# zhuduowang/Change3D

Hardware: AMD Instinct MI355X
Metric: train images/sec (256x256 pairs, X3D-L BCD) (higher is better)
Workload: dtype bf16; 1 GPU; BCD X3D-L bf16, B=32/GPU, 256x256 synthetic LEVIR-CD-shaped pairs, T=3, train step (fwd+BCE/Dice+bwd+Adam); global_batch=32, parallelism=dp1, dist_world_size=1, hip_graph=False, full=False, settle_steps=40, input=resident in HBM

## Files before the change

change3d_amd/_lib.py:

```python
import ctypes as C
import os

_HERE = os.path.dirname(os.path.abspath(__file__))
LIB_PATH = os.environ.get("C3D_LIB") or os.path.join(_HERE, "lib", "libchange3d_hip.so")

DT_F32, DT_BF16 = 0, 1
PRO_NONE, PRO_BN_SE_SWISH, PRO_AFFINE2 = 0, 1, 2
EPI_STORE, EPI_STATS, EPI_SWISH_SE_BWD, EPI_ADD = 0, 1, 2, 3
AUG_NONE, AUG_BCD, AUG_SCD, AUG_BDA = 0, 1, 2, 3
ROWS_DENSE, ROWS_FRAME, ROWS_STRIDE2, ROWS_S2SHIFT = 0, 1, 2, 3
SC_NONE, SC_IDENTITY, SC_BN, SC_RAW = 0, 1, 2, 3
STAT_STRIPES = 16
OPT_SIDE_STREAM, OPT_STEM_MFMA, OPT_CONVT_MFMA, OPT_FUSE_WGRAD, OPT_FOLD_SE, OPT_MASK_IN_DGRAD, OPT_DW_RING, OPT_PW_WGRAD_V2, OPT_DW_FWD_HV, OPT_PW_CFWD, OPT_PW_CDG, OPT_DW_T4 = 0, 1, 2, 3, 4, 5, 6, 7, 8, 9, 10, 11
STAGE_SEPARATE_FINALIZE, STAGE_NO_WEIGHT_IMAGES, STAGE_SEPARATE_RESIDUAL, STAGE_SEPARATE_WGRAD = 1, 2, 4, 8

vp, i32, i64, f32, f64 = C.c_void_p, C.c_int32, C.c_int64, C.c_float, C.c_double


class BnFin(C.Structure):
    _fields_ = [("ticket", vp), ("gamma", vp), ("beta", vp), ("running_mean", vp), ("running_var", vp), ("nbt", vp),
                ("ss", vp), ("mr", vp), ("count", f64), ("momentum", f32), ("eps", f32), ("training", i32),
                ("batch", i32), ("sums", vp)]


# ... 64 lines not shown
                ("logits_out", vp)]


SIGNATURES = {
    "c3d_abi_version": (i32, []),
    "c3d_build_info": (C.c_char_p, []),
    "c3d_device_cus": (i32, []),
    "c3d_pw_gemm": (i32, [C.POINTER(PwArgs), vp]),
    "c3d_pw_weight_image_bytes": (i64, [i32, i32, i32]),
    "c3d_pw_pack_weights": (i32, [C.POINTER(PwPackDesc), i32, i32, vp]),
    "c3d_pw_wgrad_ws_floats": (i64, [i32, i32]),
    "c3d_pw_gemm_wg_ws_floats": (i64, [i32, i32]),
    "c3d_pw_wgrad": (i32, [C.POINTER(PwWgradArgs), vp]),
    "c3d_pw_wgrad_flush": (i32, [vp]),
    "c3d_bn_finalize": (i32, [vp, i32, f64, vp, vp, vp, vp, vp, f32, f32, i32, i32, i32, vp, vp, vp]),
    "c3d_bn_se_finalize": (i32, [vp, i32, f64, vp, vp, vp, vp, vp, f32, f32, i32, i32, i32, vp, vp, vp, vp,
                                 i32, vp, vp, vp, vp, vp]),
    "c3d_bn_bwd_coef": (i32, [vp, i32, f64, vp, vp, i32, i32, vp, vp, vp, vp]),
    "c3d_se_bn_bwd_coef": (i32, [vp, vp, i32, f64, vp, vp, vp, i32, i32, vp, vp, vp, vp, i32, vp, vp, vp, vp,
                                 vp, vp, vp, vp, vp, vp]),
    "c3d_dw333_fwd": (i32, [vp, vp, vp, vp, vp, i32, i32, i32, i32, i32, i32, i32, i32, vp]),
    "c3d_dw333_fwd_fin": (i32, [vp, C.POINTER(BnFin), vp, vp, vp, i32, i32, i32, i32, i32, i32, i32, i32, vp]),
    "c3d_dw333_bwd_fused": (i32, [vp, vp, vp, vp, vp, vp, vp, vp, vp, vp, vp, vp, i32, i32, i32, i32, i32, i32, i32, i32, vp]),
    "c3d_dw333_bwd_fused_fin": (i32, [vp, vp, C.POINTER(BnFin), vp, vp, vp, vp, vp, vp, vp, i32, i32, i32, i32, i32, i32, i32, i32, vp]),
    "c3d_block_out_fwd": (i32, [vp, vp, vp, vp, i32, vp, i64, i32, i32, vp]),
    "c3d_block_out_fwd_fin": (i32, [vp, C.POINTER(BnFin), vp, C.POINTER(BnFin), i32, vp, i64, i32, i32, i32, vp]),
    "c3d_block_out_bwd": (i32, [vp, vp, vp, vp, vp, vp, vp, vp, vp, i64, i32, i32, i32, vp]),
    "c3d_block_out_bwd_fin": (i32, [vp, vp, vp, vp, vp, vp, vp, vp, vp, i64, i32, i32, i32, C.POINTER(BnFin),
                                    C.POINTER(BnFin), vp]),
    "c3d_frame_absdiff": (i32, [vp, vp, i32, i32, i64, i32, i32, i32, i32, vp]),
    "c3d_enhance_apply": (i32, [vp, vp, vp, i32, i32, i64, i32, i32, i32, vp]),
    "c3d_enhance_bwd_mask": (i32, [vp, vp, vp, i32, i32, i64, i32, i32, i32, vp]),
    "c3d_enhance_bwd_apply": (i32, [vp, vp, vp, vp, i32, i32, i64, i32, i32, i32, i32, vp]),
    "c3d_frame_scatter": (i32, [vp, vp, i32, i32, i64, i32, i32, i32, i32, vp]),
    "c3d_stem_fwd": (i32, [vp, vp, vp, vp, vp, i32, i32, i32, i32, i32, vp]),
    "c3d_stem_bwd_dv": (i32, [vp, vp, vp, vp, vp, vp, vp, vp, i32, i32, i32, i32, i32, vp]),
    "c3d_stem_bwd_wx": (i32, [vp, vp, vp, vp, vp, i32, i32, i32, i32, i32, i32, i32, i32, vp]),
    "c3d_convT4s2_fwd": (i32, [vp, vp, vp, vp, i64, vp, i32, i32, i32, i32, i32, vp]),
    "c3d_convT4s2_bwd_data": (i32, [vp, vp, vp, i32, i32, i32, i32, i32, vp]),
    "c3d_convT4s2_wgrad_ws_floats": (i64, [i32, i32, i32, i32]),
    "c3d_convT4s2_wgrad": (i32, [vp, vp, vp, vp, i32, i32, i32, i32, i32, vp]),
    "c3d_col_sum": (i32, [vp, vp, i64, i32, i32, i32, vp]),
    "c3d_head3x3_fwd": (i32, [vp, vp, vp, i32, i32, i32, i32, i32, i32, i32, vp]),
    "c3d_head3x3_bwd_ws_floats": (i64, [i32, i32, i32, i32]),
    "c3d_head3x3_bwd": (i32, [vp, vp, vp, vp, vp, vp, vp, i32, i32, i32, i32, i32, i32, i32, vp]),
    "c3d_bce_dice_fwd": (i32, [vp, vp, i64, vp, vp, vp]),
    "c3d_bce_dice_bwd": (i32, [vp, vp, vp, vp, i64, vp, vp]),
    "c3d_ce2d_fwd": (i32, [vp, vp, i64, i32, i64, i64, i64, i64, vp, vp, vp]),
    "c3d_ce2d_bwd": (i32, [vp, vp, vp, vp, i64, i32, i64, i64, i64, i64, vp, vp]),
    "c3d_cossim_fwd": (i32, [vp, vp, vp, i64, i32, i64, i64, i64, i64, i64, vp, vp, vp]),
    "c3d_cossim_bwd": (i32, [vp, vp, vp, vp, i64, i32, i64, i64, i64, i64, i64, vp, vp, vp]),
    "c3d_adam_step": (i32, [vp, vp, vp, vp, i64, vp, f32, f32, f32, f32, f32, f32, f32, vp]),
    "c3d_confusion2": (i32, [vp, vp, i64, vp, vp]),
    "c3d_hist2d": (i32, [vp, vp, i64, i32, vp, vp]),
    "c3d_bda_confusion": (i32, [vp, vp, vp, vp, i64, i32, i64, vp, vp]),
    "c3d_build_clip": (i32, [vp, vp, vp, vp, i32, i32, i32, i32, vp]),
    "c3d_bcd_preprocess": (i32, [vp, vp, vp, vp, vp, vp, vp, vp, i32, i32, i32, vp]),
    "c3d_scd_label_preprocess": (i32, [vp, vp, vp, i32, i32, i32, vp]),
    "c3d_bda_label_preprocess": (i32, [vp, vp, vp, vp, i32, i32, i32, vp]),
    "c3d_cc_preprocess": (i32, [vp, vp, vp, vp, vp, i32, i32, i32, vp]),
    "c3d_augment_gather": (i32, [vp, vp, vp, vp, vp, vp, vp, vp, vp, vp, i32, i32, i32, i32, i32, i32, i32, vp]),
    "c3d_cap_embed_fwd": (i32, [vp, vp, vp, vp, i32, i32, i32, i32, f32, C.c_uint64, i32, vp]),
    "c3d_cap_embed_bwd": (i32, [vp, vp, vp, i32, i32, i32, i32, f32, C.c_uint64, i32, vp]),
    "c3d_cap_dropout": (i32, [vp, vp, i64, i32, f32, C.c_uint64, i32, vp]),
    "c3d_cap_layernorm_fwd": (i32, [vp, vp, vp, vp, vp, vp, i64, i32, f32, i32, vp]),
    "c3d_cap_layernorm_bwd": (i32, [vp, vp, vp, vp, vp, vp, vp, vp, i64, i32, i32, vp]),
# ... 75 lines not shown
```

change3d_amd/csrc/elementwise.hip:

```cpp
#include "common.h"
#include "bn_fin.h"
#include <cstring>
#include <cstdlib>
#include <cstdlib>
#include "../../include/change3d_hip.h"

namespace {

__host__ __device__ inline int ew_block(int G) { return G * (256 / G); }

enum { SC_NONE = 0, SC_IDENTITY = 1, SC_BN = 2, SC_RAW = 3 };

template <typename T>
__global__ void block_out_fwd_kernel(const T* __restrict__ c, const float* __restrict__ ss_c,
                                     const T* __restrict__ sc, const float* __restrict__ ss_1, int sc_mode,
                                     T* __restrict__ y, int64_t nvec, int G, int C, const c3d_bn_fin fin_c,
                                     const c3d_bn_fin fin_1) {
  __shared__ float lss[4][256];
  const int v = threadIdx.x % G;
  const int Cp = G * 8;
  float a[8], b[8], a1[8], b1[8];
  if (fin_c.sums) {
    const bool owner = blockIdx.x == 0;
    if (owner && threadIdx.x == 0 && fin_c.nbt) *fin_c.nbt += 1;
// ... 162 lines not shown
    Vec8<T>::load(dout + ((b * Tn + t_mid) * hwv + r) * 8, g);
    Vec8<T>::load(e + i * 8, ev);
#pragma unroll
    for (int j = 0; j < 8; ++j) g[j] = ev[j] > 0.f ? g[j] : 0.f;
    Vec8<T>::store(de + i * 8, g);
  }
}

template <typename T>
__global__ void enhance_bwd_apply_kernel(const T* __restrict__ dout, const T* __restrict__ y,
                                         const T* __restrict__ dd, T* __restrict__ dy, int64_t nvec_all,
                                         int64_t hwv, int Tn, int t_pre, int t_post) {
  const int64_t stride = (int64_t)gridDim.x * blockDim.x;
  for (int64_t i = (int64_t)blockIdx.x * blockDim.x + threadIdx.x; i < nvec_all; i += stride) {
    const int64_t bt = i / hwv, r = i - bt * hwv;
    const int64_t b = bt / Tn;
    const int t = (int)(bt - b * Tn);
    float f[8];
    Vec8<T>::load(dout + i * 8, f);
    if (t == t_pre || t == t_post) {
      float p[8], q[8], dv[8];
      Vec8<T>::load(y + ((b * Tn + t_pre) * hwv + r) * 8, p);
      Vec8<T>::load(y + ((b * Tn + t_post) * hwv + r) * 8, q);
      Vec8<T>::load(dd + (b * hwv + r) * 8, dv);
      const float sgn_self = (t == t_pre) ? 1.f : -1.f;
#pragma unroll
      for (int j = 0; j < 8; ++j) {
        const float df = p[j] - q[j];
        const float sg = (df > 0.f) ? 1.f : ((df < 0.f) ? -1.f : 0.f);
        f[j] += sgn_self * sg * dv[j];
      }
    }
    Vec8<T>::store(dy + i * 8, f);
  }
}

template <typename T>
__global__ void frame_scatter_kernel(const T* __restrict__ src, T* __restrict__ dst, int64_t nvec, int64_t hwv,
                                     int Tn, int t_dst, int accumulate) {
  const int64_t stride = (int64_t)gridDim.x * blockDim.x;
  for (int64_t i = (int64_t)blockIdx.x * blockDim.x + threadIdx.x; i < nvec; i += stride) {
    const int64_t b = i / hwv, r = i - b * hwv;
    float f[8];
    Vec8<T>::load(src + i * 8, f);
    T* p = dst + ((b * Tn + t_dst) * hwv + r) * 8;
    if (accumulate) {
      float o[8];
      Vec8<T>::load(p, o);
#pragma unroll
      for (int j = 0; j < 8; ++j) f[j] += o[j];
    }
    Vec8<T>::store(p, f);
  }
}

inline int ew_grid(int64_t nvec, int block) {
  int64_t g = (nvec + block - 1) / block;
  if (g > 256 * 16) g = 256 * 16;
  if (g < 1) g = 1;
  return (int)g;
}

}

#define EW_DISPATCH(dtype, CALL_F32, CALL_BF16) \
  if ((dtype) == C3D_DT_F32) { CALL_F32; }      \
// ... 107 lines not shown
  return 0;
}

extern "C" int c3d_enhance_bwd_mask(const void* dout, const void* e, void* de, int32_t B, int32_t T, int64_t HW,
                                    int32_t Cp, int32_t t_mid, int32_t dtype, void* stream) {
  if (!dout || !e || !de || B <= 0 || T <= 0 || HW <= 0 || (Cp & 7) || t_mid < 0 || t_mid >= T) return C3D_E_BADARG;
  const int64_t hwv = HW * (Cp / 8), nvec = (int64_t)B * hwv;
  hipStream_t s = reinterpret_cast<hipStream_t>(stream);
  EW_DISPATCH(dtype,
              (enhance_bwd_mask_kernel<float><<<ew_grid(nvec, 256), 256, 0, s>>>((const float*)dout, (const float*)e,
                                                                                  (float*)de, nvec, hwv, T, t_mid)),
              (enhance_bwd_mask_kernel<bf16_t><<<ew_grid(nvec, 256), 256, 0, s>>>(
                  (const bf16_t*)dout, (const bf16_t*)e, (bf16_t*)de, nvec, hwv, T, t_mid)));
  C3D_CHECK_LAUNCH();
  return 0;
}

extern "C" int c3d_enhance_bwd_apply(const void* dout, const void* y, const void* dd, void* dy, int32_t B,
                                     int32_t T, int64_t HW, int32_t Cp, int32_t t_pre, int32_t t_post,
                                     int32_t dtype, void* stream) {
  if (!dout || !y || !dd || !dy || B <= 0 || T <= 0 || HW <= 0 || (Cp & 7)) return C3D_E_BADARG;
  const int64_t hwv = HW * (Cp / 8), nvec = (int64_t)B * T * hwv;
  hipStream_t s = reinterpret_cast<hipStream_t>(stream);
  EW_DISPATCH(dtype,
              (enhance_bwd_apply_kernel<float><<<ew_grid(nvec, 256), 256, 0, s>>>(
                  (const float*)dout, (const float*)y, (const float*)dd, (float*)dy, nvec, hwv, T, t_pre, t_post)),
              (enhance_bwd_apply_kernel<bf16_t><<<ew_grid(nvec, 256), 256, 0, s>>>(
                  (const bf16_t*)dout, (const bf16_t*)y, (const bf16_t*)dd, (bf16_t*)dy, nvec, hwv, T, t_pre,
                  t_post)));
  C3D_CHECK_LAUNCH();
  return 0;
}

extern "C" int c3d_frame_scatter(const void* src, void* dst, int32_t B, int32_t T, int64_t HW, int32_t Cp,
                                 int32_t t_dst, int32_t accumulate, int32_t dtype, void* stream) {
  if (!src || !dst || B <= 0 || T <= 0 || HW <= 0 || (Cp & 7) || t_dst < 0 || t_dst >= T) return C3D_E_BADARG;
  const int64_t hwv = HW * (Cp / 8), nvec = (int64_t)B * hwv;
  hipStream_t s = reinterpret_cast<hipStream_t>(stream);
  EW_DISPATCH(dtype,
              (frame_scatter_kernel<float><<<ew_grid(nvec, 256), 256, 0, s>>>((const float*)src, (float*)dst, nvec,
                                                                               hwv, T, t_dst, accumulate)),
              (frame_scatter_kernel<bf16_t><<<ew_grid(nvec, 256), 256, 0, s>>>((const bf16_t*)src, (bf16_t*)dst,
                                                                                nvec, hwv, T, t_dst, accumulate)));
  C3D_CHECK_LAUNCH();
  return 0;
}
```

change3d_amd/model/trainer.py:

```python
from typing import Any, List

import torch
import torch.nn as nn

from .. import ops
from ..ops import cpad
from .change_decoder import ChangeDecoder
from .utils import weight_init
from .x3d import _ClipStemFn, create_x3d, to_logical, to_ndhwc


class _EnhanceFn(torch.autograd.Function):

    @staticmethod
    def forward(ctx, x, weight, t_post):
        ops.require_gpu(x, "enhance input")
        B, C, T, H, W = x.shape
        act = x.dtype
        dt = ops.dt_code(act)
        dev = x.device
        xc = to_ndhwc(x.detach())
        t_mid = T // 2
        M2 = B * H * W
        d = torch.empty((M2, cpad(C)), dtype=act, device=dev)
        ops.frame_absdiff(xc, d, B, T, H * W, cpad(C), 0, t_post, dt)
        e = torch.empty_like(d)
        ops.pw_gemm(d, weight, e, M=M2, K=C, N=C, w_sn=C, w_sk=1, dtype=dt)
        out = torch.empty_like(xc)
        ops.enhance_apply(xc, e, out, B, T, H * W, cpad(C), t_mid, dt)
        ctx.saved = (xc, d, e, weight)
        ctx.meta = (B, C, T, H, W, t_post, t_mid)
        return to_logical(out)

    @staticmethod
    def backward(ctx, dout):
        xc, d, e, weight = ctx.saved
        B, C, T, H, W, t_post, t_mid = ctx.meta
        act = xc.dtype
        dt = ops.dt_code(act)
        doc = to_ndhwc(dout).to(act)
        M2 = B * H * W
        de = torch.empty_like(d)
        ops.enhance_bwd_mask(doc, e, de, B, T, H * W, cpad(C), t_mid, dt)
        dd = torch.empty_like(d)
        ops.pw_gemm(de, weight, dd, M=M2, K=C, N=C, w_sn=1, w_sk=C, dtype=dt)
        gw = ops.grad_of(weight)
        ops.side_run(lambda: ops.pw_wgrad(de, d, gw, M=M2, K=C, N=C, dw_sn=C, dw_sk=1, dtype=dt), de, d)
        dx = torch.empty_like(xc)
        ops.enhance_bwd_apply(doc, xc, dd, dx, B, T, H * W, cpad(C), 0, t_post, dt)
        return to_logical(dx), None, None


def _ndhwc_storage(t):
    p = t.permute(0, 2, 3, 4, 1)
    return p if p.is_contiguous() else None


TAP_INPLACE = True


class _TapFrames(torch.autograd.Function):

    @staticmethod
    def forward(ctx, x, k0, n):
        ctx.set_materialize_grads(False)
        ctx.k0, ctx.n, ctx.x_meta = k0, n, (tuple(x.shape), x.dtype)
        return (x.view_as(x),) + tuple(x[:, :, k0 + i] for i in range(n))

    @staticmethod
    def backward(ctx, gx, *gf):
        (B, C, T, H, W), act = ctx.x_meta
        live = [(i, g) for i, g in enumerate(gf) if g is not None]
        if gx is None and not live:
            return None, None, None
        dev = (gx if gx is not None else live[0][1]).device
        dt = ops.dt_code(act)
        fresh = gx is None
        own = TAP_INPLACE and (not fresh) and gx.dtype == act and not gx.requires_grad and gx.grad_fn is None
        buf = _ndhwc_storage(gx) if own else None
        if buf is None:
            buf = torch.empty((B, T, H, W, C), dtype=act, device=dev)
            if fresh:
                tapped = {ctx.k0 + i for i, _ in live}
# ... 8 lines not shown
                gc = gc.to(act).contiguous()
            ops.frame_scatter(gc, buf, B, T, H * W, C, ctx.k0 + i, 0 if fresh else 1, dt)
        return buf.permute(0, 4, 1, 2, 3), None, None


def tap_frames(x, k0, n):
    out = _TapFrames.apply(x, k0, n)
    return out[0], list(out[1:])


class Encoder(nn.Module):

    def __init__(self, args: Any, embed_dims: List[int]) -> None:
        super().__init__()
        self.args = args
        act_dtype = getattr(args, "act_dtype", torch.float32)
        self.x3d = create_x3d(input_clip_length=3, depth_factor=5.0, act_dtype=act_dtype)
        try:
            state_dict = torch.load(args.pretrained, map_location="cpu")["model_state"]
            msg = self.x3d.load_state_dict(state_dict, strict=True)
            print(f"Load pretrained weight: {args.pretrained}, {msg}.")
        except Exception as e:
            print(f"Failed to load pretrained weights: {e}")
        self.perception_frames = nn.Parameter(
            torch.randn(1, 3, args.num_perception_frame, args.in_height, args.in_width), requires_grad=True)
        self.fc = nn.ModuleList([
            nn.Sequential(nn.Conv2d(dim, dim, kernel_size=1, stride=1, padding=0, bias=False), nn.ReLU())
            for dim in embed_dims])
        self.x3d.blocks[0].grad_frames = (1, args.num_perception_frame)

    def enhance(self, x: torch.Tensor, fc: nn.Module) -> torch.Tensor:
        return _EnhanceFn.apply(x, fc[0].weight, self.args.num_perception_frame + 1)

    def base_forward(self, x: torch.Tensor, output_final: bool = False, _stem_out=None):
        if output_final:
            for i in range(5):
                x = _stem_out if (i == 0 and _stem_out is not None) else self.x3d.blocks[i](x)
            return x[:, :, self.args.num_perception_frame]
        out = []
        for i in range(4):
            x = _stem_out if (i == 0 and _stem_out is not None) else self.x3d.blocks[i](x)
            x = self.enhance(x, self.fc[i])
            x, frames = tap_frames(x, 1, self.args.num_perception_frame)
            out.append(frames)
        return out

    def forward(self, x: torch.Tensor, y: torch.Tensor, output_final: bool = False):
        stem = self.x3d.blocks[0]
        if (x.is_cuda and not x.requires_grad and not y.requires_grad and x.dim() == 4 and x.shape[1] == 3
                and (x.shape[2] * x.shape[3]) % 4 == 0 and tuple(x.shape[2:]) == tuple(self.perception_frames.shape[3:])):
            s0 = _ClipStemFn.apply(x, y, self.perception_frames, stem.norm.weight, stem)
            return self.base_forward(None, output_final, _stem_out=s0)
        expand = self.perception_frames.expand(x.shape[0], -1, -1, -1, -1)
        frames = torch.cat([x.unsqueeze(2), expand, y.unsqueeze(2)], dim=2)
        return self.base_forward(frames, output_final)


class Trainer(nn.Module):

    def __init__(self, args: Any) -> None:
        super().__init__()
        self.args = args
        self.embed_dims = [24, 24, 48, 96]
        self.encoder = Encoder(args, self.embed_dims)
        k = args.num_perception_frame
        if k == 1 and "CD" in args.dataset:
            self.decoder = ChangeDecoder(args, in_dim=self.embed_dims, has_sigmoid=True)
            weight_init(self.decoder)
        elif k == 3:
            self.decoder_pre = ChangeDecoder(args, in_dim=self.embed_dims)
            self.decoder_post = ChangeDecoder(args, in_dim=self.embed_dims)
            self.decoder_change = ChangeDecoder(args, in_dim=self.embed_dims, has_sigmoid=True)
            weight_init(self.decoder_pre)
            weight_init(self.decoder_post)
            weight_init(self.decoder_change)
        elif k == 2:
            self.decoder_cls = ChangeDecoder(args, in_dim=self.embed_dims)
            self.decoder_loc = ChangeDecoder(args, in_dim=self.embed_dims, has_sigmoid=True)
            weight_init(self.decoder_cls)
            weight_init(self.decoder_loc)
        elif k == 1 and "CC" in args.dataset:
            from .caption_decoder import CaptionDecoder
            self.decoder = CaptionDecoder(args)
# ... 25 lines not shown
```

change3d_amd/model/x3d.py:

```python
import math

import os

import torch
import torch.nn as nn

from .. import ops
from ..ops import cpad

BN_EPS, BN_MOM = 1e-5, 0.1


def round_width(width, multiplier, min_width=8, divisor=8, ceil=False):
    if not multiplier:
        return width
    width *= multiplier
    min_width = min_width or divisor
    if ceil:
        out = max(min_width, int(math.ceil(width / divisor)) * divisor)
    else:
        out = max(min_width, int(width + divisor / 2) // divisor * divisor)
    if out < 0.9 * width:
        out += divisor
    return int(out)


def round_repeats(repeats, multiplier):
    return repeats if not multiplier else int(math.ceil(multiplier * repeats))


def to_ndhwc(x):
    return x.permute(0, 2, 3, 4, 1).contiguous()


def to_logical(y):
    return y.permute(0, 4, 1, 2, 3)


class _Holder(nn.Module):
    """Plain container; keeps attribute names identical to the reference module tree."""


def _f32(n, dev):
    return torch.empty(n, dtype=torch.float32, device=dev)


def _stem_forward(ctx, xin, stem):
    B, Ci, T, H, W = xin.shape
    dev, dt = xin.device, ops.dt_code(stem.act_dtype)
    training = stem.training
    conv_s, conv_t = stem.conv.conv_t, stem.conv.conv_xy
    C = conv_s.weight.shape[0]
    sums = torch.zeros(2 * C, dtype=torch.float64, device=dev) if training else None
    u = torch.empty((B, T, H, W, C), dtype=stem.act_dtype, device=dev)
    ops.stem_fwd(xin, conv_s.weight, conv_t.weight, u, sums, B, T, H, W, dt)
    ss, mr = _f32(2 * cpad(C), dev), _f32(2 * cpad(C), dev)
    ops.bn_finalize(sums, B * T * H * W, stem.norm, C, ss, mr, training)
    y = torch.empty_like(u)
    ops.block_out_fwd(u, ss, None, None, ops.SC_NONE, y, B * T * H * W, cpad(C), dt)
    ctx.stem, ctx.saved = stem, (xin, u, y, mr)
    return to_logical(y)


def _stem_backward(ctx, dy, frames_grad=None):
    stem = ctx.stem
    xin, u, y, mr = ctx.saved
    B, _, T, H, W = xin.shape
    dev, dt = xin.device, ops.dt_code(stem.act_dtype)
    conv_s, conv_t = stem.conv.conv_t, stem.conv.conv_xy
    C = conv_s.weight.shape[0]
    M = B * T * H * W
    dyc = to_ndhwc(dy).to(stem.act_dtype)
    g = torch.empty_like(u)
    dsums = torch.zeros(2 * C, dtype=torch.float64, device=dev)
    ops.block_out_bwd(dyc, y, u, None, g, mr, None, dsums, None, M, C, dt)
    coef = _f32(3 * cpad(C), dev)
    ops.bn_bwd_coef(dsums, M, stem.norm, mr, C, coef)
    dv = torch.empty_like(u)
    ops.stem_bwd_dv(xin, conv_s.weight, conv_t.weight, g, u, coef, dv, ops.grad_of(conv_t.weight), B, T, H, W, dt)
    dx = None
    if frames_grad is not None:
        gp, t0, nf = frames_grad
        ops.stem_bwd_wx(xin, conv_s.weight, dv, ops.grad_of(conv_s.weight), gp, B, T, H, W, t0, nf, False, dt)
    elif ctx.x_needs_grad:
        t0, nf = stem.grad_frames if stem.grad_frames is not None else (0, T)
        dx = torch.zeros_like(xin)
        ops.stem_bwd_wx(xin, conv_s.weight, dv, ops.grad_of(conv_s.weight), dx, B, T, H, W, t0, nf, True, dt)
    else:
        ops.stem_bwd_wx(xin, conv_s.weight, dv, ops.grad_of(conv_s.weight), None, B, T, H, W, 0, 0, False, dt)
    return dx


class _StemFn(torch.autograd.Function):
    @staticmethod
    def forward(ctx, x, anchor, stem):
        ops.require_gpu(x, "stem input")
        if x.shape[1] != 3:
            raise NotImplementedError("stem kernel is specialised for 3 input channels")
        ctx.x_needs_grad = x.requires_grad
        return _stem_forward(ctx, x.detach().contiguous().float(), stem)

    @staticmethod
    def backward(ctx, dy):
        return _stem_backward(ctx, dy), None, None


class _ClipStemFn(torch.autograd.Function):

# ... 351 lines not shown
```

change3d_amd/ops.py:

```python
import ctypes as C

import os

import torch

from . import _lib as L
from ._lib import (OPT_CONVT_MFMA, OPT_DW_FWD_HV, OPT_DW_RING, OPT_DW_T4, OPT_FOLD_SE, OPT_FUSE_WGRAD, OPT_MASK_IN_DGRAD, OPT_PW_CDG, OPT_PW_CFWD, OPT_PW_WGRAD_V2, OPT_SIDE_STREAM, OPT_STEM_MFMA, STAGE_NO_WEIGHT_IMAGES, STAGE_SEPARATE_FINALIZE,
                   STAGE_SEPARATE_RESIDUAL, STAGE_SEPARATE_WGRAD)
from ._lib import (DT_BF16, DT_F32, EPI_ADD, EPI_STATS, EPI_STORE, EPI_SWISH_SE_BWD, PRO_AFFINE2,
                   PRO_BN_SE_SWISH, PRO_NONE, ROWS_DENSE, ROWS_FRAME, ROWS_S2SHIFT, ROWS_STRIDE2, SC_BN,
                   SC_IDENTITY, SC_NONE, SC_RAW, STAT_STRIPES)


def cpad(c):
    return (c + 7) // 8 * 8


def dt_code(dtype):
    if dtype == torch.float32:
        return DT_F32
    if dtype == torch.bfloat16:
        return DT_BF16
    raise TypeError(f"unsupported activation dtype {dtype} (float32 | bfloat16)")

# ... 352 lines not shown
                                      _stream())


def block_out_fwd_fin(c, fin_c, shortcut, fin_1, mode, y, M, C_, dtype):
    _launch("c3d_block_out_fwd", M * cpad(C_) * (3 if shortcut is not None else 2) * _es(dtype), L.lib().c3d_block_out_fwd_fin, _p(c), C.byref(fin_c), _p(shortcut),
                                      C.byref(fin_1) if fin_1 is not None else None, mode, _p(y), M, C_, cpad(C_), dtype, _stream())


def block_out_bwd(dy, y, c, s_bn, g, mr_c, mr_1, dsums_c, dsums_1, M, C_, dtype):
    _launch("c3d_block_out_bwd", M * cpad(C_) * (5 if s_bn is not None else 4) * _es(dtype), L.lib().c3d_block_out_bwd, _p(dy), _p(y), _p(c), _p(s_bn), _p(g), _p(mr_c), _p(mr_1), _p(dsums_c), _p(dsums_1), M, C_,
                                      cpad(C_), dtype, _stream())


def block_out_bwd_fin(dy, y, c, s_bn, g, mr_c, mr_1, dsums_c, dsums_1, M, C_, dtype, fin_c, fin_1):
    _launch("c3d_block_out_bwd", M * cpad(C_) * (5 if s_bn is not None else 4) * _es(dtype), L.lib().c3d_block_out_bwd_fin, _p(dy), _p(y), _p(c), _p(s_bn), _p(g), _p(mr_c), _p(mr_1), _p(dsums_c), _p(dsums_1), M, C_,
            cpad(C_), dtype, C.byref(fin_c), C.byref(fin_1) if fin_1 is not None else None, _stream())


def frame_absdiff(y, d, B, T, HW, Cp, t_pre, t_post, dtype):
    _launch("c3d_frame_absdiff", B * HW * Cp * 3 * _es(dtype), L.lib().c3d_frame_absdiff, _p(y), _p(d), B, T, HW, Cp, t_pre, t_post, dtype, _stream())


def enhance_apply(y, e, out, B, T, HW, Cp, t_mid, dtype):
    _launch("c3d_enhance_apply", B * HW * Cp * (2 * T + 1) * _es(dtype), L.lib().c3d_enhance_apply, _p(y), _p(e), _p(out), B, T, HW, Cp, t_mid, dtype, _stream())


def enhance_bwd_mask(dout, e, de, B, T, HW, Cp, t_mid, dtype):
    _launch("c3d_enhance_bwd_mask", B * HW * Cp * 3 * _es(dtype), L.lib().c3d_enhance_bwd_mask, _p(dout), _p(e), _p(de), B, T, HW, Cp, t_mid, dtype, _stream())


def enhance_bwd_apply(dout, y, dd, dy, B, T, HW, Cp, t_pre, t_post, dtype):
    _launch("c3d_enhance_bwd_apply", B * HW * Cp * (2 * T + 3) * _es(dtype), L.lib().c3d_enhance_bwd_apply, _p(dout), _p(y), _p(dd), _p(dy), B, T, HW, Cp, t_pre, t_post, dtype,
                                          _stream())


def frame_scatter(src, dst, B, T, HW, Cp, t_dst, accumulate, dtype):
    _launch("c3d_frame_scatter", B * HW * Cp * (3 if accumulate else 2) * _es(dtype), L.lib().c3d_frame_scatter, _p(src), _p(dst), B, T, HW, Cp,
            t_dst, 1 if accumulate else 0, dtype, _stream())


def stem_fwd(x, w_t, w_xy, u, sums, B, T, H, W, dtype):
    _launch("c3d_stem_fwd", x.numel() * 4 + u.numel() * _es(dtype), L.lib().c3d_stem_fwd, _p(x), _p(w_t), _p(w_xy), _p(u), _p(sums), B, T, H, W, dtype, _stream())


def stem_bwd_dv(x, w_t, w_xy, g0, u, coef, dv, dw_xy, B, T, H, W, dtype):
    _launch("c3d_stem_bwd_dv", x.numel() * 4 + 3 * u.numel() * _es(dtype), L.lib().c3d_stem_bwd_dv, _p(x), _p(w_t), _p(w_xy), _p(g0), _p(u), _p(coef), _p(dv), _p(dw_xy), B, T, H,
                                    W, dtype, _stream())


def stem_bwd_wx(x, w_t, dv, dw_t, dP, B, T, H, W, t_first, n_frames, per_sample, dtype):
    _launch("c3d_stem_bwd_wx", x.numel() * 4 + dv.numel() * _es(dtype), L.lib().c3d_stem_bwd_wx, _p(x), _p(w_t), _p(dv), _p(dw_t), _p(dP), B, T, H, W, t_first, n_frames,
                                    1 if per_sample else 0, dtype, _stream())


def convT_fwd(inp, w, bias, skip_ptr, skip_bstride, out, B, h, wd, C_, dtype):
    _launch("c3d_convT4s2_fwd", (inp.numel() + 2 * out.numel()) * _es(dtype), L.lib().c3d_convT4s2_fwd, _p(inp), _p(w), _p(bias), skip_ptr, skip_bstride, _p(out), B, h, wd, C_,
                                     dtype, _stream())


def convT_bwd_data(dout, w, din, B, h, wd, C_, dtype):
    _launch("c3d_convT4s2_bwd_data", (dout.numel() + din.numel()) * _es(dtype), L.lib().c3d_convT4s2_bwd_data, _p(dout), _p(w), _p(din), B, h, wd, C_, dtype, _stream())


CONVT_MFMA = os.environ.get("C3D_CONVT_MFMA", "1") != "0"


# ... 330 lines not shown
```

include/change3d_hip.h:

```cpp
#ifndef CHANGE3D_HIP_H
#define CHANGE3D_HIP_H
#include <stdint.h>

#ifdef __cplusplus
extern "C" {
#endif

#define C3D_DT_F32 0
#define C3D_DT_BF16 1

#define C3D_E_BADARG (-1)
#define C3D_E_UNSUPPORTED (-2)

int c3d_abi_version(void);
const char* c3d_build_info(void);
int c3d_device_cus(void);

#define C3D_PRO_NONE 0
#define C3D_PRO_BN_SE_SWISH 1
#define C3D_PRO_AFFINE2 2

#define C3D_EPI_STORE 0
#define C3D_EPI_STATS 1
#define C3D_STAT_STRIPES 16
// ... 125 lines not shown
int c3d_dw333_fwd_fin(const void* x, const c3d_bn_fin* fin, const float* w, void* y, double* nc_sums, int32_t B,
                      int32_t T, int32_t H, int32_t W, int32_t C, int32_t Cp, int32_t stride, int32_t dtype,
                      void* stream);
int c3d_dw333_bwd_fused(const void* t1, const void* b, const float* coefA, const float* coefB,
                        const float* coefC, const float* w, const void* a, const float* ss_a,
                        const float* mr_a, void* t2, double* dsums, float* dw, int32_t B, int32_t T,
                        int32_t H, int32_t W, int32_t C, int32_t Cp, int32_t stride, int32_t dtype, void* stream);
int c3d_dw333_bwd_fused_fin(const void* t1, const void* b, const c3d_bn_fin* fin_b, const float* w, const void* a,
                            const float* ss_a, const float* mr_a, void* t2, double* dsums, float* dw, int32_t B,
                            int32_t T, int32_t H, int32_t W, int32_t C, int32_t Cp, int32_t stride, int32_t dtype,
                            void* stream);

int c3d_block_out_fwd(const void* c, const float* ss_c, const void* shortcut, const float* ss_1,
                      int32_t sc_mode, void* y, int64_t M, int32_t Cp, int32_t dtype, void* stream);
int c3d_block_out_fwd_fin(const void* c, const c3d_bn_fin* fin_c, const void* shortcut, const c3d_bn_fin* fin_1,
                          int32_t sc_mode, void* y, int64_t M, int32_t C, int32_t Cp, int32_t dtype, void* stream);
int c3d_block_out_bwd(const void* dy, const void* y, const void* c, const void* s_bn, void* g,
                      const float* mr_c, const float* mr_1, double* dsums_c, double* dsums_1, int64_t M,
                      int32_t C, int32_t Cp, int32_t dtype, void* stream);
int c3d_block_out_bwd_fin(const void* dy, const void* y, const void* c, const void* s_bn, void* g,
                          const float* mr_c, const float* mr_1, double* dsums_c, double* dsums_1, int64_t M,
                          int32_t C, int32_t Cp, int32_t dtype, const c3d_bn_fin* fin_c, const c3d_bn_fin* fin_1,
                          void* stream);

int c3d_frame_absdiff(const void* y, void* d, int32_t B, int32_t T, int64_t HW, int32_t Cp, int32_t t_pre,
                      int32_t t_post, int32_t dtype, void* stream);
int c3d_enhance_apply(const void* y, const void* e, void* out, int32_t B, int32_t T, int64_t HW,
                      int32_t Cp, int32_t t_mid, int32_t dtype, void* stream);
int c3d_enhance_bwd_mask(const void* dout, const void* e, void* de, int32_t B, int32_t T, int64_t HW,
                         int32_t Cp, int32_t t_mid, int32_t dtype, void* stream);
int c3d_enhance_bwd_apply(const void* dout, const void* y, const void* dd, void* dy, int32_t B, int32_t T,
                          int64_t HW, int32_t Cp, int32_t t_pre, int32_t t_post, int32_t dtype,
                          void* stream);
int c3d_frame_scatter(const void* src, void* dst, int32_t B, int32_t T, int64_t HW, int32_t Cp,
                      int32_t t_dst, int32_t accumulate, int32_t dtype, void* stream);

int c3d_stem_fwd(const float* x, const float* w_t, const float* w_xy, void* u, double* sums, int32_t B,
                 int32_t T, int32_t H, int32_t W, int32_t dtype, void* stream);
int c3d_stem_bwd_dv(const float* x, const float* w_t, const float* w_xy, const void* g0, const void* u,
                    const float* coef, void* dv, float* dw_xy, int32_t B, int32_t T, int32_t H, int32_t W,
                    int32_t dtype, void* stream);
int c3d_stem_bwd_wx(const float* x, const float* w_t, const void* dv, float* dw_t, float* dP, int32_t B,
                    int32_t T, int32_t H, int32_t W, int32_t t_first, int32_t n_frames, int32_t per_sample,
                    int32_t dtype, void* stream);

int c3d_convT4s2_fwd(const void* in, const float* w, const float* bias, const void* skip,
                     int64_t skip_bstride, void* out, int32_t B, int32_t h, int32_t wd, int32_t C,
                     int32_t dtype, void* stream);
int c3d_convT4s2_bwd_data(const void* dout, const float* w, void* din, int32_t B, int32_t h, int32_t wd,
                          int32_t C, int32_t dtype, void* stream);
int64_t c3d_convT4s2_wgrad_ws_floats(int32_t B, int32_t h, int32_t wd, int32_t C);
int c3d_convT4s2_wgrad(const void* t, const void* dout, float* dw, float* ws, int32_t B, int32_t h, int32_t wd,
                       int32_t C, int32_t dtype, void* stream);
int c3d_col_sum(const void* x, float* out, int64_t M, int32_t C, int32_t Cp, int32_t dtype, void* stream);
int c3d_head3x3_fwd(const void* x, const float* w, float* out, int32_t B, int32_t H, int32_t W, int32_t C,
                    int32_t NC, int32_t has_sigmoid, int32_t dtype, void* stream);
int64_t c3d_head3x3_bwd_ws_floats(int32_t B, int32_t H, int32_t W, int32_t NC);
int c3d_head3x3_bwd(const float* dout, const float* prob, const void* x, const float* w, void* dx,
                    float* dw, float* ws, int32_t B, int32_t H, int32_t W, int32_t C, int32_t NC, int32_t has_sigmoid,
                    int32_t dtype, void* stream);

int c3d_bce_dice_fwd(const float* prob, const float* target, int64_t n, double* sums4, float* loss,
                     void* stream);
int c3d_bce_dice_bwd(const float* prob, const float* target, const double* sums4, const float* dloss,
                     int64_t n, float* dprob, void* stream);
int c3d_adam_step(float* param, const float* grad, float* exp_avg, float* exp_avg_sq, int64_t n,
// ... 153 lines not shown
```

Before: 1598 images/s.

## Fuse stem BN/ReLU output with first-stage enhance in forward and backward

Adds fused kernels that apply the stem's BN affine and ReLU on the fly and combine them with the stage-0 enhance step: abs-diff of the pre/post frames, the mid-frame add of relu(e), and a backward kernel that merges the enhance sign-gradient, the ReLU mask and the BN dsums reduction. A new autograd function is used by default in training. The aim is to stop materialising the stem output y and the separate enhance passes, which removes several full-tensor HBM reads and writes. In exchange the backward recomputes y from u, which adds some arithmetic, and the code paths for the stem are now more complex.

```diff
diff --git a/change3d_amd/_lib.py b/change3d_amd/_lib.py
--- a/change3d_amd/_lib.py
+++ b/change3d_amd/_lib.py
@@ -120,6 +120,9 @@
     "c3d_enhance_apply": (i32, [vp, vp, vp, i32, i32, i64, i32, i32, i32, vp]),
     "c3d_enhance_bwd_mask": (i32, [vp, vp, vp, i32, i32, i64, i32, i32, i32, vp]),
     "c3d_enhance_bwd_apply": (i32, [vp, vp, vp, vp, i32, i32, i64, i32, i32, i32, i32, vp]),
+    "c3d_stem_enhance_fwd": (i32, [vp, vp, vp, vp, i32, i32, i64, i32, i32, i32, i32, i32, vp]),
+    "c3d_stem_enhance_mid": (i32, [vp, vp, vp, vp, i32, i32, i64, i32, i32, i32, vp]),
+    "c3d_stem_enhance_bwd": (i32, [vp, vp, vp, vp, vp, vp, vp, i32, i32, i64, i32, i32, i32, i32, i32, vp]),
     "c3d_frame_scatter": (i32, [vp, vp, i32, i32, i64, i32, i32, i32, i32, vp]),
     "c3d_stem_fwd": (i32, [vp, vp, vp, vp, vp, i32, i32, i32, i32, i32, vp]),
     "c3d_stem_bwd_dv": (i32, [vp, vp, vp, vp, vp, vp, vp, vp, i32, i32, i32, i32, i32, vp]),
diff --git a/change3d_amd/csrc/elementwise.hip b/change3d_amd/csrc/elementwise.hip
--- a/change3d_amd/csrc/elementwise.hip
+++ b/change3d_amd/csrc/elementwise.hip
@@ -218,6 +218,178 @@
       }
     }
     Vec8<T>::store(dy + i * 8, f);
+  }
+}
+
+template <typename T>
+__device__ __forceinline__ void stem_y(const float (&uv)[8], const float (&a)[8], const float (&b)[8], float (&y)[8]) {
+#pragma unroll
+  for (int j = 0; j < 8; ++j) y[j] = round_as<T>(fmaxf(fmaf(uv[j], a[j], b[j]), 0.f));
+}
+
+__device__ __forceinline__ void load_rows8(const float* __restrict__ p, float (&f)[8]) {
+  const float4 x = *reinterpret_cast<const float4*>(p), y = *reinterpret_cast<const float4*>(p + 4);
+  f[0] = x.x; f[1] = x.y; f[2] = x.z; f[3] = x.w; f[4] = y.x; f[5] = y.y; f[6] = y.z; f[7] = y.w;
+}
+
+template <typename T>
+__global__ __launch_bounds__(256) void stem_enhance_fwd_kernel(const T* __restrict__ u, const float* __restrict__ ss,
+                                                               T* __restrict__ out, T* __restrict__ d, int64_t nvec,
+                                                               int64_t hwv, int G, int Tn, int t_pre, int t_post,
+                                                               int t_mid) {
+  const int v = threadIdx.x % G;
+  float a[8], b[8];
+  load_rows8(ss + v * 8, a);
+  load_rows8(ss + G * 8 + v * 8, b);
+  typedef typename Vec8<T>::raw_t raw_t;
+  const int64_t stride = (int64_t)gridDim.x * blockDim.x;
+  for (int64_t i = (int64_t)blockIdx.x * blockDim.x + threadIdx.x; i < nvec; i += stride) {
+    const int64_t bb = i / hwv, r = i - bb * hwv;
+    const int64_t base = bb * Tn * hwv + r;
+    const raw_t rp = Vec8<T>::load_raw(u + (base + t_pre * hwv) * 8);
+    const raw_t rq = Vec8<T>::load_raw(u + (base + t_post * hwv) * 8);
+    float f[8], p[8], q[8];
+    Vec8<T>::cvt_raw(rp, f);
+    stem_y<T>(f, a, b, p);
+    Vec8<T>::store(out + (base + t_pre * hwv) * 8, p);
+    Vec8<T>::cvt_raw(rq, f);
+    stem_y<T>(f, a, b, q);
+    Vec8<T>::store(out + (base + t_post * hwv) * 8, q);
+#pragma unroll
+    for (int j = 0; j < 8; ++j) p[j] = fabsf(p[j] - q[j]);
+    Vec8<T>::store(d + i * 8, p);
+    for (int t = 0; t < Tn; ++t) {
+      if (t == t_pre || t == t_post || t == t_mid) continue;
+      Vec8<T>::load(u + (base + t * hwv) * 8, f);
+      stem_y<T>(f, a, b, q);
+      Vec8<T>::store(out + (base + t * hwv) * 8, q);
+    }
+  }
+}
+
+template <typename T>
+__global__ __launch_bounds__(256) void stem_enhance_mid_kernel(const T* __restrict__ u, const float* __restrict__ ss,
+                                                               const T* __restrict__ e, T* __restrict__ out,
+                                                               int64_t nvec, int64_t hwv, int G, int Tn, int t_mid) {
+  const int v = threadIdx.x % G;
+  float a[8], b[8];
+  load_rows8(ss + v * 8, a);
+  load_rows8(ss + G * 8 + v * 8, b);
+  typedef typename Vec8<T>::raw_t raw_t;
+  const int64_t stride = (int64_t)gridDim.x * blockDim.x;
+  for (int64_t i = (int64_t)blockIdx.x * blockDim.x + threadIdx.x; i < nvec; i += stride) {
+    const int64_t bb = i / hwv, r = i - bb * hwv;
+    const int64_t row = (bb * Tn + t_mid) * hwv + r;
+    const raw_t ru = Vec8<T>::load_raw(u + row * 8);
+    const raw_t re = Vec8<T>::load_raw(e + i * 8);
+    float f[8], y[8], ev[8];
+    Vec8<T>::cvt_raw(ru, f);
+    Vec8<T>::cvt_raw(re, ev);
+    stem_y<T>(f, a, b, y);
+#pragma unroll
+    for (int j = 0; j < 8; ++j) y[j] += fmaxf(ev[j], 0.f);
+    Vec8<T>::store(out + row * 8, y);
+  }
+}
+
+template <typename T>
+__global__ __launch_bounds__(256) void stem_enhance_bwd_kernel(const T* __restrict__ dout, const T* __restrict__ c,
+                                                               const float* __restrict__ ss, const T* __restrict__ dd,
+                                                               T* __restrict__ g, const float* __restrict__ mr_c,
+                                                               double* __restrict__ dsums_c, int64_t nvec, int64_t hwv,
+                                                               int G, int C, int Tn, int t_pre, int t_post) {
+  extern __shared__ float red[];
+  const int v = threadIdx.x % G;
+  const int Cp = G * 8;
+  float s1[8], s2[8];
+  float mc[8], rc[8], a[8], b[8];
+  load_rows8(mr_c + v * 8, mc);
+  load_rows8(mr_c + Cp + v * 8, rc);
+  load_rows8(ss + v * 8, a);
+  load_rows8(ss + Cp + v * 8, b);
+#pragma unroll
+  for (int j = 0; j < 8; ++j) { s1[j] = 0.f; s2[j] = 0.f; }
+  const int64_t stride = (int64_t)gridDim.x * blockDim.x;
+  const int64_t other = (int64_t)(t_post - t_pre) * hwv;
+  constexpr int BOB_U = 4;
+  typedef typename Vec8<T>::raw_t raw_t;
+  int64_t ci = (int64_t)blockIdx.x * blockDim.x + threadIdx.x;
+  int64_t cb, cr;
+  int ct;
+  {
+    const int64_t bt = ci / hwv;
+    cr = ci - bt * hwv;
+    cb = bt / Tn;
+    ct = (int)(bt - cb * Tn);
+  }
+  for (int64_t i0 = ci; i0 < nvec; i0 += BOB_U * stride) {
+    raw_t rd[BOB_U], rc_[BOB_U], ro[BOB_U], rdd[BOB_U];
+    int side[BOB_U];
+#pragma unroll
+    for (int u = 0; u < BOB_U; ++u) {
+      const int64_t i = i0 + u * stride;
+      side[u] = 0;
+      if (i < nvec) {
+        rd[u] = Vec8<T>::load_raw(dout + i * 8);
+        rc_[u] = Vec8<T>::load_raw(c + i * 8);
+        side[u] = (ct == t_pre) ? 1 : ((ct == t_post) ? -1 : 0);
+        if (side[u]) {
+          ro[u] = Vec8<T>::load_raw(c + (i + side[u] * other) * 8);
+          rdd[u] = Vec8<T>::load_raw(dd + (cb * hwv + cr) * 8);
+        }
+        cr += stride;
+        while (cr >= hwv) {
+          cr -= hwv;
+          if (++ct == Tn) { ct = 0; ++cb; }
+        }
+      }
+    }
+#pragma unroll
+    for (int u = 0; u < BOB_U; ++u) {
+      const int64_t i = i0 + u * stride;
+      if (i < nvec) {
+        float d[8], yv[8], cv[8];
+        Vec8<T>::cvt_raw(rd[u], d);
+        Vec8<T>::cvt_raw(rc_[u], cv);
+        stem_y<T>(cv, a, b, yv);
+        if (side[u]) {
+          float ov[8], yo[8], dv[8];
+          Vec8<T>::cvt_raw(ro[u], ov);
+          Vec8<T>::cvt_raw(rdd[u], dv);
+          stem_y<T>(ov, a, b, yo);
+          const float sgn_self = (side[u] > 0) ? 1.f : -1.f;
+#pragma unroll
+          for (int j = 0; j < 8; ++j) {
+            const float df = (side[u] > 0) ? (yv[j] - yo[j]) : (yo[j] - yv[j]);
+            const float sg = (df > 0.f) ? 1.f : ((df < 0.f) ? -1.f : 0.f);
+            d[j] = round_as<T>(d[j] + sgn_self * sg * dv[j]);
+          }
+        }
+#pragma unroll
+        for (int j = 0; j < 8; ++j) {
+          const float gg = (yv[j] > 0.f) ? d[j] : 0.f;
+          d[j] = gg;
+          s1[j] += gg; s2[j] += gg * ((cv[j] - mc[j]) * rc[j]);
+        }
+        Vec8<T>::store(g + i * 8, d);
+      }
+    }
+  }
+#pragma unroll
+  for (int j = 0; j < 8; ++j) {
+    red[threadIdx.x * 24 + j] = s1[j]; red[threadIdx.x * 24 + 8 + j] = s2[j]; red[threadIdx.x * 24 + 16 + j] = 0.f;
+  }
+  __syncthreads();
+  for (int idx = threadIdx.x; idx < G * 24; idx += blockDim.x) {
+    const int vv = idx / 24, k = idx % 24;
+    double acc = 0;
+    for (int t = vv; t < (int)blockDim.x; t += G) acc += red[t * 24 + k];
+    const int ch = vv * 8 + (k & 7);
+    const int which = k >> 3;
+    if (ch < C) {
+      if (which == 0) atomicAdd(dsums_c + ch, acc);
+      else if (which == 1) atomicAdd(dsums_c + C + ch, acc);
+    }
   }
 }
 
@@ -391,6 +563,74 @@
   return 0;
 }
 
+namespace {
+inline bool stem_enhance_geom_ok(int32_t B, int32_t T, int64_t HW, int32_t Cp, int32_t t_pre, int32_t t_post, int32_t t_mid) {
+  if (B <= 0 || T < 3 || HW <= 0 || Cp <= 0 || (Cp & 7) || Cp > 256) return false;
+  if (t_pre < 0 || t_pre >= T || t_post < 0 || t_post >= T || t_mid < 0 || t_mid >= T) return false;
+  return t_pre != t_post && t_mid != t_pre && t_mid != t_post;
+}
+}
+
+extern "C" int c3d_stem_enhance_fwd(const void* u, const float* ss, void* out, void* d, int32_t B, int32_t T, int64_t HW,
+                                    int32_t Cp, int32_t t_pre, int32_t t_post, int32_t t_mid, int32_t dtype, void* stream) {
+  if (!u || !ss || !out || !d || !stem_enhance_geom_ok(B, T, HW, Cp, t_pre, t_post, t_mid)) return C3D_E_BADARG;
+  if ((uintptr_t)ss & 15) return C3D_E_BADARG;
+  const int G = Cp / 8, blk = ew_block(G);
+  const int64_t hwv = HW * G, nvec = (int64_t)B * hwv;
+  hipStream_t s = reinterpret_cast<hipStream_t>(stream);
+  EW_DISPATCH(dtype,
+              (stem_enhance_fwd_kernel<float><<<ew_grid(nvec, blk), blk, 0, s>>>(
+                  (const float*)u, ss, (float*)out, (float*)d, nvec, hwv, G, T, t_pre, t_post, t_mid)),
+              (stem_enhance_fwd_kernel<bf16_t><<<ew_grid(nvec, blk), blk, 0, s>>>(
+                  (const bf16_t*)u, ss, (bf16_t*)out, (bf16_t*)d, nvec, hwv, G, T, t_pre, t_post, t_mid)));
+  C3D_CHECK_LAUNCH();
+  return 0;
+}
+
+extern "C" int c3d_stem_enhance_mid(const void* u, const float* ss, const void* e, void* out, int32_t B, int32_t T,
+                                    int64_t HW, int32_t Cp, int32_t t_mid, int32_t dtype, void* stream) {
+  if (!u || !ss || !e || !out || B <= 0 || T <= 0 || HW <= 0 || Cp <= 0 || (Cp & 7) || Cp > 256 || t_mid < 0 || t_mid >= T)
+    return C3D_E_BADARG;
+  if ((uintptr_t)ss & 15) return C3D_E_BADARG;
+  const int G = Cp / 8, blk = ew_block(G);
+  const int64_t hwv = HW * G, nvec = (int64_t)B * hwv;
+  hipStream_t s = reinterpret_cast<hipStream_t>(stream);
+  EW_DISPATCH(dtype,
+              (stem_enhance_mid_kernel<float><<<ew_grid(nvec, blk), blk, 0, s>>>(
+                  (const float*)u, ss, (const float*)e, (float*)out, nvec, hwv, G, T, t_mid)),
+              (stem_enhance_mid_kernel<bf16_t><<<ew_grid(nvec, blk), blk, 0, s>>>(
+                  (const bf16_t*)u, ss, (const bf16_t*)e, (bf16_t*)out, nvec, hwv, G, T, t_mid)));
+  C3D_CHECK_LAUNCH();
+  return 0;
+}
+
+extern "C" int c3d_stem_enhance_bwd(const void* dout, const void* u, const float* ss, const void* dd, const float* mr,
+                                    void* g, double* dsums, int32_t B, int32_t T, int64_t HW, int32_t C, int32_t Cp,
+                                    int32_t t_pre, int32_t t_post, int32_t dtype, void* stream) {
+  if (!dout || !u || !ss || !dd || !mr || !g || !dsums || C <= 0 || C > Cp) return C3D_E_BADARG;
+  if (B <= 0 || T < 2 || HW <= 0 || (Cp & 7) || Cp > 256 || t_pre < 0 || t_pre >= T || t_post < 0 || t_post >= T ||
+      t_pre == t_post)
+    return C3D_E_BADARG;
+  if (((uintptr_t)ss & 15) || ((uintptr_t)mr & 15)) return C3D_E_BADARG;
+  const int G = Cp / 8, blk = ew_block(G);
+  const int64_t hwv = HW * G, nvec = (int64_t)B * T * hwv;
+  int grid = ew_grid(nvec, blk);
+  static const int env_cap = c3d_env("C3D_BOB_GRID") ? atoi(c3d_env("C3D_BOB_GRID")) : 0;
+  const int cap = env_cap > 0 ? env_cap : 384;
+  if (grid > cap) grid = cap;
+  const size_t lds = (size_t)blk * 24 * sizeof(float);
+  hipStream_t s = reinterpret_cast<hipStream_t>(stream);
+  EW_DISPATCH(dtype,
+              (stem_enhance_bwd_kernel<float><<<grid, blk, lds, s>>>((const float*)dout, (const float*)u, ss,
+                                                                      (const float*)dd, (float*)g, mr, dsums, nvec, hwv, G,
+                                                                      C, T, t_pre, t_post)),
+              (stem_enhance_bwd_kernel<bf16_t><<<grid, blk, lds, s>>>((const bf16_t*)dout, (const bf16_t*)u, ss,
+                                                                       (const bf16_t*)dd, (bf16_t*)g, mr, dsums, nvec, hwv,
+                                                                       G, C, T, t_pre, t_post)));
+  C3D_CHECK_LAUNCH();
+  return 0;
+}
+
 extern "C" int c3d_frame_scatter(const void* src, void* dst, int32_t B, int32_t T, int64_t HW, int32_t Cp,
                                  int32_t t_dst, int32_t accumulate, int32_t dtype, void* stream) {
   if (!src || !dst || B <= 0 || T <= 0 || HW <= 0 || (Cp & 7) || t_dst < 0 || t_dst >= T) return C3D_E_BADARG;
diff --git a/change3d_amd/model/trainer.py b/change3d_amd/model/trainer.py
--- a/change3d_amd/model/trainer.py
+++ b/change3d_amd/model/trainer.py
@@ -7,7 +7,7 @@
 from ..ops import cpad
 from .change_decoder import ChangeDecoder
 from .utils import weight_init
-from .x3d import _ClipStemFn, create_x3d, to_logical, to_ndhwc
+from .x3d import _ClipStemFn, _stem_backward_convs, _stem_forward_convs, create_x3d, to_logical, to_ndhwc
 
 
 class _EnhanceFn(torch.autograd.Function):
@@ -49,6 +49,59 @@
         dx = torch.empty_like(xc)
         ops.enhance_bwd_apply(doc, xc, dd, dx, B, T, H * W, cpad(C), 0, t_post, dt)
         return to_logical(dx), None, None
+
+
+class _ClipStemEnhanceFn(torch.autograd.Function):
+
+    @staticmethod
+    def forward(ctx, pre, post, frames, anchor, stem, weight, t_post):
+        ops.require_gpu(pre, "encoder input")
+        B, Ci, H, W = pre.shape
+        K = frames.shape[2]
+        if Ci != 3 or tuple(frames.shape) != (1, 3, K, H, W) or tuple(post.shape) != tuple(pre.shape):
+            raise NotImplementedError("clip assembly expects (B,3,H,W) images and (1,3,K,H,W) perception frames")
+        T = K + 2
+        clip = torch.empty((B, 3, T, H, W), dtype=torch.float32, device=pre.device)
+        ops.build_clip(pre.detach().contiguous().float(), post.detach().contiguous().float(),
+                       frames.detach().contiguous().float(), clip, B, K, H, W)
+        act, dt = stem.act_dtype, ops.dt_code(stem.act_dtype)
+        u, ss, mr = _stem_forward_convs(clip, stem)
+        C = u.shape[-1]
+        t_mid, M2 = T // 2, B * H * W
+        out = torch.empty_like(u)
+        d = torch.empty((M2, cpad(C)), dtype=act, device=u.device)
+        ops.stem_enhance_fwd(u, ss, out, d, B, T, H * W, cpad(C), 0, t_post, t_mid, dt)
+        e = torch.empty_like(d)
+        ops.pw_gemm(d, weight, e, M=M2, K=C, N=C, w_sn=C, w_sk=1, dtype=dt)
+        ops.stem_enhance_mid(u, ss, e, out, B, T, H * W, cpad(C), t_mid, dt)
+        ctx.stem, ctx.frames, ctx.K, ctx.x_needs_grad = stem, frames, K, False
+        ctx.need_frames = ctx.needs_input_grad[2]
+        ctx.saved = (clip, u, ss, mr, d, e, weight)
+        ctx.meta = (t_post, t_mid)
+        return to_logical(out)
+
+    @staticmethod
+    def backward(ctx, dout):
+        clip, u, ss, mr, d, e, weight = ctx.saved
+        t_post, t_mid = ctx.meta
+        B, T, H, W, C = u.shape
+        act, dt = u.dtype, ops.dt_code(u.dtype)
+        doc = to_ndhwc(dout).to(act)
+        M2 = B * H * W
+        de = torch.empty_like(d)
+        ops.enhance_bwd_mask(doc, e, de, B, T, H * W, cpad(C), t_mid, dt)
+        dd = torch.empty_like(d)
+        ops.pw_gemm(de, weight, dd, M=M2, K=C, N=C, w_sn=1, w_sk=C, dtype=dt)
+        gw = ops.grad_of(weight)
+        ops.side_run(lambda: ops.pw_wgrad(de, d, gw, M=M2, K=C, N=C, dw_sn=C, dw_sk=1, dtype=dt), de, d)
+        g = torch.empty_like(u)
+        dsums = torch.zeros(2 * C, dtype=torch.float64, device=u.device)
+        ops.stem_enhance_bwd(doc, u, ss, dd, mr, g, dsums, B, T, H * W, C, 0, t_post, dt)
+        gp = None
+        if ctx.need_frames:
+            gp = torch.zeros(ctx.frames.shape, dtype=torch.float32, device=dout.device)
+        _stem_backward_convs(ctx, clip, u, mr, g, dsums, (gp, 1, ctx.K) if gp is not None else None)
+        return None, None, gp, None, None, None, None
 
 
 def _ndhwc_storage(t):
@@ -123,7 +176,7 @@
     def enhance(self, x: torch.Tensor, fc: nn.Module) -> torch.Tensor:
         return _EnhanceFn.apply(x, fc[0].weight, self.args.num_perception_frame + 1)
 
-    def base_forward(self, x: torch.Tensor, output_final: bool = False, _stem_out=None):
+    def base_forward(self, x: torch.Tensor, output_final: bool = False, _stem_out=None, _stem_enhanced=False):
         if output_final:
             for i in range(5):
                 x = _stem_out if (i == 0 and _stem_out is not None) else self.x3d.blocks[i](x)
@@ -131,15 +184,23 @@
         out = []
         for i in range(4):
             x = _stem_out if (i == 0 and _stem_out is not None) else self.x3d.blocks[i](x)
-            x = self.enhance(x, self.fc[i])
+            if not (i == 0 and _stem_out is not None and _stem_enhanced):
+                x = self.enhance(x, self.fc[i])
             x, frames = tap_frames(x, 1, self.args.num_perception_frame)
             out.append(frames)
         return out
 
+    def _clip_stem_ok(self, x: torch.Tensor, y: torch.Tensor) -> bool:
+        return (x.is_cuda and not x.requires_grad and not y.requires_grad and x.dim() == 4 and x.shape[1] == 3
+                and (x.shape[2] * x.shape[3]) % 4 == 0 and tuple(x.shape[2:]) == tuple(self.perception_frames.shape[3:]))
+
     def forward(self, x: torch.Tensor, y: torch.Tensor, output_final: bool = False):
         stem = self.x3d.blocks[0]
-        if (x.is_cuda and not x.requires_grad and not y.requires_grad and x.dim() == 4 and x.shape[1] == 3
-                and (x.shape[2] * x.shape[3]) % 4 == 0 and tuple(x.shape[2:]) == tuple(self.perception_frames.shape[3:])):
+        if self._clip_stem_ok(x, y):
+            if ops.STEM_ENHANCE and not output_final:
+                s0 = _ClipStemEnhanceFn.apply(x, y, self.perception_frames, stem.norm.weight, stem, self.fc[0][0].weight,
+                                              self.args.num_perception_frame + 1)
+                return self.base_forward(None, output_final, _stem_out=s0, _stem_enhanced=True)
             s0 = _ClipStemFn.apply(x, y, self.perception_frames, stem.norm.weight, stem)
             return self.base_forward(None, output_final, _stem_out=s0)
         expand = self.perception_frames.expand(x.shape[0], -1, -1, -1, -1)
diff --git a/change3d_amd/model/x3d.py b/change3d_amd/model/x3d.py
--- a/change3d_amd/model/x3d.py
+++ b/change3d_amd/model/x3d.py
@@ -45,7 +45,7 @@
     return torch.empty(n, dtype=torch.float32, device=dev)
 
 
-def _stem_forward(ctx, xin, stem):
+def _stem_forward_convs(xin, stem):
     B, Ci, T, H, W = xin.shape
     dev, dt = xin.device, ops.dt_code(stem.act_dtype)
     training = stem.training
@@ -56,6 +56,14 @@
     ops.stem_fwd(xin, conv_s.weight, conv_t.weight, u, sums, B, T, H, W, dt)
     ss, mr = _f32(2 * cpad(C), dev), _f32(2 * cpad(C), dev)
     ops.bn_finalize(sums, B * T * H * W, stem.norm, C, ss, mr, training)
+    return u, ss, mr
+
+
+def _stem_forward(ctx, xin, stem):
+    B, Ci, T, H, W = xin.shape
+    dt = ops.dt_code(stem.act_dtype)
+    C = stem.conv.conv_t.weight.shape[0]
+    u, ss, mr = _stem_forward_convs(xin, stem)
     y = torch.empty_like(u)
     ops.block_out_fwd(u, ss, None, None, ops.SC_NONE, y, B * T * H * W, cpad(C), dt)
     ctx.stem, ctx.saved = stem, (xin, u, y, mr)
@@ -74,6 +82,16 @@
     g = torch.empty_like(u)
     dsums = torch.zeros(2 * C, dtype=torch.float64, device=dev)
     ops.block_out_bwd(dyc, y, u, None, g, mr, None, dsums, None, M, C, dt)
+    return _stem_backward_convs(ctx, xin, u, mr, g, dsums, frames_grad)
+
+
+def _stem_backward_convs(ctx, xin, u, mr, g, dsums, frames_grad=None):
+    stem = ctx.stem
+    B, _, T, H, W = xin.shape
+    dev, dt = xin.device, ops.dt_code(stem.act_dtype)
+    conv_s, conv_t = stem.conv.conv_t, stem.conv.conv_xy
+    C = conv_s.weight.shape[0]
+    M = B * T * H * W
     coef = _f32(3 * cpad(C), dev)
     ops.bn_bwd_coef(dsums, M, stem.norm, mr, C, coef)
     dv = torch.empty_like(u)
diff --git a/change3d_amd/ops.py b/change3d_amd/ops.py
--- a/change3d_amd/ops.py
+++ b/change3d_amd/ops.py
@@ -408,6 +408,24 @@
 def enhance_bwd_apply(dout, y, dd, dy, B, T, HW, Cp, t_pre, t_post, dtype):
     _launch("c3d_enhance_bwd_apply", B * HW * Cp * (2 * T + 3) * _es(dtype), L.lib().c3d_enhance_bwd_apply, _p(dout), _p(y), _p(dd), _p(dy), B, T, HW, Cp, t_pre, t_post, dtype,
                                           _stream())
+
+
+STEM_ENHANCE = os.environ.get("C3D_STEM_ENHANCE", "1") != "0"
+
+
+def stem_enhance_fwd(u, ss, out, d, B, T, HW, Cp, t_pre, t_post, t_mid, dtype):
+    _launch("c3d_stem_enhance_fwd", B * HW * Cp * (2 * T - 1) * _es(dtype), L.lib().c3d_stem_enhance_fwd, _p(u), _p(ss), _p(out), _p(d),
+            B, T, HW, Cp, t_pre, t_post, t_mid, dtype, _stream())
+
+
+def stem_enhance_mid(u, ss, e, out, B, T, HW, Cp, t_mid, dtype):
+    _launch("c3d_stem_enhance_mid", B * HW * Cp * 3 * _es(dtype), L.lib().c3d_stem_enhance_mid, _p(u), _p(ss), _p(e), _p(out),
+            B, T, HW, Cp, t_mid, dtype, _stream())
+
+
+def stem_enhance_bwd(dout, u, ss, dd, mr, g, dsums, B, T, HW, C_, t_pre, t_post, dtype):
+    _launch("c3d_stem_enhance_bwd", B * HW * cpad(C_) * (3 * T + 1) * _es(dtype), L.lib().c3d_stem_enhance_bwd, _p(dout), _p(u), _p(ss),
+            _p(dd), _p(mr), _p(g), _p(dsums), B, T, HW, C_, cpad(C_), t_pre, t_post, dtype, _stream())
 
 
 def frame_scatter(src, dst, B, T, HW, Cp, t_dst, accumulate, dtype):
diff --git a/include/change3d_hip.h b/include/change3d_hip.h
--- a/include/change3d_hip.h
+++ b/include/change3d_hip.h
@@ -181,6 +181,13 @@
 int c3d_enhance_bwd_apply(const void* dout, const void* y, const void* dd, void* dy, int32_t B, int32_t T,
                           int64_t HW, int32_t Cp, int32_t t_pre, int32_t t_post, int32_t dtype,
                           void* stream);
+int c3d_stem_enhance_fwd(const void* u, const float* ss, void* out, void* d, int32_t B, int32_t T, int64_t HW,
+                         int32_t Cp, int32_t t_pre, int32_t t_post, int32_t t_mid, int32_t dtype, void* stream);
+int c3d_stem_enhance_mid(const void* u, const float* ss, const void* e, void* out, int32_t B, int32_t T, int64_t HW,
+                         int32_t Cp, int32_t t_mid, int32_t dtype, void* stream);
+int c3d_stem_enhance_bwd(const void* dout, const void* u, const float* ss, const void* dd, const float* mr, void* g,
+                         double* dsums, int32_t B, int32_t T, int64_t HW, int32_t C, int32_t Cp, int32_t t_pre,
+                         int32_t t_post, int32_t dtype, void* stream);
 int c3d_frame_scatter(const void* src, void* dst, int32_t B, int32_t T, int64_t HW, int32_t Cp,
                       int32_t t_dst, int32_t accumulate, int32_t dtype, void* stream);
 
```

Result: faster. 1635 images/s (median of 6 runs) (+2.3%).
